# valette/FROG

Hardware: AMD Instinct MI355X
Metric: registration iterations/sec (linear+deformable) (higher is better)
Workload: dtype f32

## Files before the change

### frog_amd/csrc/device/frog_hip.hip

```cpp

#include "ctx.h"
#include <hip/hip_ext.h>
#include "prep.h"
#include "k_links.hip.h"
#include "k_stats.hip.h"
#include "k_grid.hip.h"
#include "k_cull.hip.h"
#include "k_ransac.hip.h"
#include "k_reforder.hip.h"
#include "k_refchain.hip.h"
#include "similarity.h"

#include <atomic>
#include <chrono>
#include <cmath>
#include <cstdlib>
#include <random>
#include <limits>
#include <new>

namespace frog {
thread_local std::string g_last_error;
constexpr int BOUNDS_BLOCKS = 256;
void set_last_error(const std::string &s) { g_last_error = s; }
}

using namespace frog;

#define CTX_GUARD(ctx)                                                   \
    do {                                                                 \
        if (!(ctx)) return fail(FROG_E_INVALID, "null context");         \
        FROG_HIP_CHECK(hipSetDevice((ctx)->device));                      \
    } while (0)

__attribute__((constructor)) static void frog_openmp_defaults()
{
    setenv("KMP_AFFINITY", "disabled", 0);
    setenv("KMP_BLOCKTIME", "0", 0);
}

static inline unsigned div_up(size_t a, size_t b) { return (unsigned)((a + b - 1) / b); }

#include <dlfcn.h>
namespace {
struct Roctx {
    int (*push)(const char *) = nullptr;
    int (*pop)() = nullptr;
    Roctx()
    {
        const char *e = getenv("FROG_ROCTX");
        if (!e || !atoi(e)) return;
        for (const char *name : { "librocprofiler-sdk-roctx.so", "librocprofiler-sdk-roctx.so.1", "libroctx64.so", "libroctx64.so.4" }) {
            if (void *h = dlopen(name, RTLD_NOW | RTLD_GLOBAL)) {
                push = (int (*)(const char *))dlsym(h, "roctxRangePushA");
                pop = (int (*)())dlsym(h, "roctxRangePop");
                if (push && pop) return;
                push = nullptr; pop = nullptr;
            }
        }
    }
};
const Roctx &roctx() { static Roctx r; return r; }
const char *const K_GROUP_NAMES[FROG_K_COUNT_] = { "frog:sweep_linear", "frog:sweep_deformable", "frog:scatter", "frog:lattice_step", "frog:transform_points",
                                                    "frog:update_stats", "frog:combine_energy", "frog:cull_check", "frog:sweep_deformable_build_list",
                                                    "frog:sweep_linear_build_list" };
}

struct Span {
    frog_ctx *c; int slot; hipEvent_t a = nullptr, b = nullptr;
    bool attached;
    bool range = false;
    Span(frog_ctx *ctx, int s, bool attach = false) : c(ctx), slot(s), attached(attach)
    {
        if (roctx().push) { roctx().push(K_GROUP_NAMES[s]); range = true; }
        if (!c->profiling || (c->profiling == 2 && s > FROG_K_SWEEP_DEFORMABLE && s != FROG_K_SWEEP_BUILD && s != FROG_K_SWEEP_LINEAR_BUILD)) return;
        const uint64_t seen = c->span_seen[s]++;
        if (c->profiling == 2 && c->profile_stride > 1 && (s == FROG_K_SWEEP_DEFORMABLE || s == FROG_K_SWEEP_LINEAR) && seen % (uint64_t)c->profile_stride != 0) return;
        if (!c->free_events.empty()) { a = c->free_events.back().first; b = c->free_events.back().second; c->free_events.pop_back(); }
        else if (hipEventCreate(&a) != hipSuccess || hipEventCreate(&b) != hipSuccess) { a = b = nullptr; return; }
        if (!attached) (void)hipEventRecord(a, c->stream);
    }
    ~Span()
    {
        if (a) {
            if (!attached) (void)hipEventRecord(b, c->stream);
            c->spans.push_back({ a, b, slot });
        }
        if (range) roctx().pop();
    }
};

template <class T> static int download_points(frog_ctx *ctx, const T *src, float *dst)
{
    std::vector<T> h(ctx->P);
    FROG_HIP_CHECK(hipMemcpyAsync(h.data(), src, h.size() * sizeof(T), hipMemcpyDeviceToHost, ctx->stream));
    FROG_HIP_CHECK(hipStreamSynchronize(ctx->stream));
    for (size_t p = 0; p < ctx->P; p++) {
        const T &v = h[ctx->h_new_of_old[p]];
        dst[3 * p] = v.x; dst[3 * p + 1] = v.y; dst[3 * p + 2] = v.z;
    }
    return FROG_OK;
}

static unsigned sweep_blocks(const frog_ctx *ctx) { return div_up(ctx->n_tiles, 4) * N_XCD; }

static_assert(THRESHOLD_BAND == 1e-4f, "ctx.h frog_ctx::fast_theta spells the band out");

static uint32_t sweep_lds_images(const frog_ctx *ctx)
{
    if (ctx->rec_format.narrow) return 1u << ctx->rec_format.img_bits;
    uint32_t widest = 0;
    for (uint32_t g = 0; g < ctx->n_groups; g++) widest = std::max(widest, ctx->group_begin[g + 1] - ctx->group_begin[g]);
    return widest <= (uint32_t)EMD_LDS_IMAGES ? widest : 0u;
}

static SweepArgs sweep_args(frog_ctx *ctx, uint32_t sub)
{
    SweepArgs a;
    a.sub = sub;
    a.n_groups = ctx->n_groups;
    for (uint32_t g = 0; g <= ctx->n_groups; g++) a.group_begin[g] = ctx->group_begin[g];
    a.tiles = ctx->tiles.p; a.recs = ctx->rec_format.narrow ? (const void *)ctx->recs32.p : (const void *)ctx->recs.p; a.pos2 = ctx->pos2.p; a.emd = ctx->emd.p; a.emf = ctx->emf.p; a.em = ctx->em.p;
    a.rec2_last = (uint32_t)(ctx->L_recs / 2 - 1);
    a.img_bits = ctx->rec_format.img_bits; a.lds_images = sweep_lds_images(ctx); a.poff = ctx->d_poff.p; a.point_last = (uint32_t)(ctx->P ? ctx->P - 1 : 0);
    a.n_tiles = ctx->n_tiles; a.threshold = ctx->opt.inlier_threshold;
    a.band = ctx->exact_weights ? __builtin_inff() : THRESHOLD_BAND;
    a.tile_partial = ctx->tile_partial.p; a.tile_counts = ctx->tile_counts.p; a.group_sums = ctx->group_sums.p;
    a.own_pt_begin = ctx->own_pt_begin; a.own_points = ctx->own_pt_end - ctx->own_pt_begin;
    a.act_recs = nullptr; a.act_cnt = nullptr; a.cull_state = nullptr;
    a.cut_list = nullptr; a.build_recs = nullptr; a.build_cnt = nullptr;
    a.point_sums = ctx->point_sums.p; a.tile_order = ctx->tile_order.p; a.tiles_bo = ctx->tiles_bo.p;
    return a;
}

static bool cull_active(const frog_ctx *ctx)
{
    return ctx->cull_enabled && ctx->deformable && ctx->opt.inlier_threshold >= 1e-3f && ctx->n_tiles > 0;
}

static bool cull_active_linear(const frog_ctx *ctx)
{
    return ctx->cull_enabled && ctx->cull_linear && !ctx->exact_weights && !ctx->deformable && ctx->n_tiles > 0 && ctx->n_sub == 1;
}

static bool sweep_builds_list(const frog_ctx *ctx) { return ctx->rec_format.narrow != 0; }

static bool sweep_fused_now(const frog_ctx *ctx, bool build)
{
    return ctx->fused_sweep && !build;
}

template <int MODE>
static void launch_sweep(frog_ctx *ctx, uint32_t sub, hipStream_t s, hipEvent_t ea = nullptr, hipEvent_t eb = nullptr,
                         bool use_list = false, bool build_list = false)
{
    uint32_t widest = 0;
    for (uint32_t g = 0; g < ctx->n_groups; g++) widest = std::max(widest, ctx->group_begin[g + 1] - ctx->group_begin[g]);
    if (ctx->n_tiles == 0) return;
    SweepArgs args = sweep_args(ctx, sub);
    if (use_list) {
        args.act_recs = ctx->rec_format.narrow ? (const void *)ctx->act_recs32.p : (const void *)ctx->act_recs.p;
        args.act_cnt = ctx->act_cnt.p;
        args.cull_state = ctx->cull_state.p;
    }
    const dim3 grid(sweep_blocks(ctx)), block(256);
    const size_t lds = (size_t)args.lds_images * (sizeof(EmDerived) + sizeof(uint32_t) + sizeof(float));
    if constexpr (MODE == SWEEP_LINEAR) {
        if (build_list && sweep_builds_list(ctx)) {
            args.act_recs = nullptr; args.act_cnt = nullptr;
            args.cut_list = ctx->cut_list.p; args.build_recs = ctx->act_recs32.p; args.build_cnt = ctx->act_cnt.p;
            hipExtLaunchKernelGGL((sweep_kernel<SWEEP_LINEAR, true, false, true>), grid, block, lds, s, ea, eb, 0, args);
            return;
        }
    }
    if constexpr (MODE == SWEEP_DEFORMABLE) {
        const bool build = build_list && sweep_builds_list(ctx);
        if (build) {
            args.act_recs = nullptr; args.act_cnt = nullptr;
            args.cut_list = ctx->cut_list.p; args.build_recs = ctx->act_recs32.p; args.build_cnt = ctx->act_cnt.p;
        }
        if (sweep_fused_now(ctx, build)) {
            const dim3 fgrid(ctx->n_order_blocks), fblock(512);
            const size_t flds = lds * N_XCD;
            if (ctx->rec_format.narrow) hipExtLaunchKernelGGL((sweep_kernel<SWEEP_DEFORMABLE, true, false, false, true>), fgrid, fblock, flds, s, ea, eb, 0, args);
            else hipExtLaunchKernelGGL((sweep_kernel<SWEEP_DEFORMABLE, true, true, false, true>), fgrid, fblock, flds, s, ea, eb, 0, args);
            return;
        }
        if (build) {
            hipExtLaunchKernelGGL((sweep_kernel<SWEEP_DEFORMABLE, true, false, true>), grid, block, lds, s, ea, eb, 0, args);
            return;
        }
    }
    if (ctx->rec_format.narrow)
        hipExtLaunchKernelGGL((sweep_kernel<MODE, true, false>), grid, block, lds, s, ea, eb, 0, args);
    else if (widest <= (uint32_t)EMD_LDS_IMAGES)
        hipExtLaunchKernelGGL((sweep_kernel<MODE, true, true>), grid, block, lds, s, ea, eb, 0, args);
    else
        hipExtLaunchKernelGGL((sweep_kernel<MODE, false, true>), grid, block, 0, s, ea, eb, 0, args);
}

static int cull_allocate(frog_ctx *ctx);
static int cull_prepare(frog_ctx *ctx);
static int make_geometry(const frog_ctx *ctx, int level, const double mins[3], const double maxs[3], GridGeom &g, frog_grid_info &info);
static int lattice_alloc(frog_ctx *ctx, const GridGeom &g);

__global__ void scratch_warm_kernel(unsigned int *out, int n)
{
    volatile unsigned int a[16];
    for (int k = 0; k < 16; k++) a[k] = (unsigned int)(k * n);
    unsigned int v = 0;
    for (int k = 0; k < 16; k++) v += a[(k + n) & 15];
    if (n < 0) out[0] = v;
}

static uint32_t scatter_max_blocks(uint32_t n_bricks_total, uint32_t n_points, uint32_t chunk)
{
    return std::min(n_bricks_total, n_points) + n_points / chunk;
}

static int queue_setup_kernels(frog_ctx *ctx, hipStream_t s)
{
    const GridGeom &g = ctx->geom;
    const uint32_t nO = ctx->n_owned();
    const uint32_t nPts = ctx->own_pt_end - ctx->own_pt_begin;
    const size_t nb = (size_t)g.n_bricks;
    int rc = FROG_OK;
    {
        ZeroList z{};
        auto add = [&](void *p, size_t bytes) {
            if (!p || !bytes) return;
            z.p[z.n] = (uint32_t *)p; z.bytes[z.n] = bytes;
            z.first_block[z.n + 1] = z.first_block[z.n] + (unsigned)((bytes + ZERO_BLOCK_BYTES - 1) / ZERO_BLOCK_BYTES);
            z.n++;
        };
        add(ctx->gradf.p, ctx->gradf.bytes()); add(ctx->coeff.p, ctx->coeff.bytes()); add(ctx->grad.p, ctx->grad.bytes());
        add(ctx->gridsum.p, ctx->gridsum.bytes()); add(ctx->key_counts.p, ctx->key_counts.bytes());
        add(ctx->len_hist.p, ctx->len_hist.bytes());
        if (g.sparse) {
            add(ctx->lat_mask.p, ctx->lat_mask.bytes()); add(ctx->ucoeff.p, ctx->ucoeff.bytes()); add(ctx->ugrad.p, ctx->ugrad.bytes());
            add(ctx->ugrad_spare.p, ctx->ugrad_spare.bytes());
        }
        if (z.n) {
            zero_buffers_kernel<<<z.first_block[z.n], 256, 0, s>>>(z);
            FROG_HIP_CHECK(hipGetLastError());
        }
    }

    const uint32_t keys_per_brick = (uint32_t)(g.brick * g.brick * g.brick);
    const uint32_t n_keys = (uint32_t)((size_t)nO * nb * keys_per_brick);
    const uint32_t n_bricks_total = nO * (uint32_t)nb;
    frog::DevBuf<uint32_t> &counts = ctx->key_counts, &chunks = ctx->brick_ptr_scratch;
    const GeomDev gd = to_dev(g);
    uint32_t max_img_pts = 0;
    for (uint32_t i = ctx->ib; i < ctx->ie; i++) max_img_pts = std::max(max_img_pts, ctx->poff[i + 1] - ctx->poff[i]);
    const dim3 bgrid(std::max(1u, div_up(max_img_pts, BRICK_BLOCK_POINTS)), nO);
    if (nPts) {
        brick_count_kernel<<<bgrid, 256, 0, s>>>(ctx->pos.p, ctx->d_poff.p, ctx->ib, gd, counts.p);
        FROG_HIP_CHECK(hipGetLastError());
    }
    auto exclusive_scan = [&](const uint32_t *in, uint32_t n, uint32_t *ptr, uint32_t *cursor) -> int {
        const uint32_t n_scan_blocks = div_up(n, SCAN_BLOCK_ITEMS);
        frog::DevBuf<uint32_t> &bsums = ctx->scan_sums;
        scan_block_sums_kernel<<<n_scan_blocks, 1024, 0, s>>>(in, n, bsums.p);
        scan_of_sums_kernel<<<1, 1024, 0, s>>>(bsums.p, n_scan_blocks, bsums.p + n_scan_blocks);
        scan_apply_kernel<<<n_scan_blocks, 1024, 0, s>>>(in, n, bsums.p, bsums.p + n_scan_blocks, ptr, cursor);
        FROG_HIP_CHECK(hipGetLastError());
        return FROG_OK;
    };
    rc = exclusive_scan(counts.p, n_keys, ctx->key_ptr.p, ctx->key_cursor.p);
    if (rc) return rc;
    if (nPts) {
        brick_place_kernel<<<bgrid, 256, 0, s>>>(ctx->pos.p, ctx->d_poff.p, ctx->ib, gd, ctx->key_cursor.p, ctx->perm.p, ctx->perm_key.p);
        FROG_HIP_CHECK(hipGetLastError());
        cell_order_kernel<<<div_up(nPts, 256), 256, 0, s>>>(ctx->key_ptr.p, ctx->perm_key.p, nPts, ctx->perm.p, ctx->perm_tmp.p);
        FROG_HIP_CHECK(hipGetLastError());
        std::swap(ctx->perm.p, ctx->perm_tmp.p);
        std::swap(ctx->perm.cap, ctx->perm_tmp.cap);
        std::swap(ctx->perm.n, ctx->perm_tmp.n);
        gather_positions_kernel<<<div_up(nPts, 256), 256, 0, s>>>(ctx->pos.p, ctx->perm.p, nPts, ctx->pos_b.p);
        FROG_HIP_CHECK(hipGetLastError());
        ctx->pos_b_stale = false;
    }
    const uint32_t max_blocks = scatter_max_blocks(n_bricks_total, nPts, SCATTER_CHUNK);
    brick_chunks_kernel<<<div_up(n_bricks_total, 256), 256, 0, s>>>(ctx->key_ptr.p, n_bricks_total, keys_per_brick, SCATTER_CHUNK, chunks.p);
    FROG_HIP_CHECK(hipGetLastError());
    rc = exclusive_scan(chunks.p, n_bricks_total, ctx->brick_slot_ptr.p, ctx->key_cursor.p );
    if (rc) return rc;
    ScatterBlock *blk_tmp = reinterpret_cast<ScatterBlock *>(ctx->scatter_blocks_tmp.p);
    ScatterBlock *blk = reinterpret_cast<ScatterBlock *>(ctx->scatter_blocks.p);
    uint32_t *len_hist = ctx->len_hist.p, *len_cursor = ctx->len_hist.p + (SCATTER_CHUNK + 1);
    const uint32_t *n_blocks_dev = ctx->brick_slot_ptr.p + n_bricks_total;
    block_fill_kernel<<<div_up(n_bricks_total, 256), 256, 0, s>>>(ctx->key_ptr.p, ctx->brick_slot_ptr.p, n_bricks_total, keys_per_brick,
                                                                 SCATTER_CHUNK, blk_tmp, len_hist);
    static_assert(SCATTER_CHUNK + 1 <= 1024, "block_len_base_kernel: one thread per block length");
    block_len_base_kernel<<<1, (SCATTER_CHUNK + 1 + 63) / 64 * 64, 0, s>>>(len_hist, len_cursor);
    if (max_blocks)
        block_sort_kernel<<<div_up(max_blocks, 256), 256, 0, s>>>(blk_tmp, n_blocks_dev, SCATTER_CHUNK, len_cursor, blk);
    if (g.sparse) {
        if (nPts && max_blocks) lattice_mask_kernel<<<max_blocks, 64, 0, s>>>(ctx->pos_b.p, blk, n_blocks_dev, gd, ctx->lat_mask.p);
        lattice_inactive_kernel<<<div_up((size_t)gd.n_cp, 256), 256, 0, s>>>(ctx->lat_mask.p, nO, gd, ctx->lat_inactive.p);
    }
    FROG_HIP_CHECK(hipGetLastError());
    return FROG_OK;
}

static int join_setup(frog_ctx *ctx)
{
    if (ctx->setup_deferred) {
        ctx->setup_deferred = false;
        FROG_HIP_CHECK(hipStreamWaitEvent(ctx->setup_stream, ctx->setup_fork, 0));
        const int rc = queue_setup_kernels(ctx, ctx->setup_stream);
        if (rc) return rc;
        FROG_HIP_CHECK(hipEventRecord(ctx->setup_join, ctx->setup_stream));
        ctx->setup_pending = true;
    }
    if (!ctx->setup_pending) return FROG_OK;
    FROG_HIP_CHECK(hipStreamWaitEvent(ctx->stream, ctx->setup_join, 0));
    ctx->setup_pending = false;
    return FROG_OK;
}

static int join_setup_positions(frog_ctx *ctx)
{
    const int rc = join_setup(ctx);
    if (rc) return rc;
    const uint32_t nPts = ctx->own_pt_end - ctx->own_pt_begin;
    if (ctx->pos_b_stale && nPts && ctx->pos_b.p && ctx->perm.p) {
        gather_positions_kernel<<<div_up(nPts, 256), 256, 0, ctx->stream>>>(ctx->pos.p, ctx->perm.p, nPts, ctx->pos_b.p);
        FROG_HIP_CHECK(hipGetLastError());
        ctx->pos_b_stale = false;
    }
    return FROG_OK;
}

static int wait_step_scalars(frog_ctx *ctx, double seq)
{
    volatile double *h = ctx->h_energy;
    const auto t0 = std::chrono::steady_clock::now();
    unsigned spins = 0;
    while (h[7] != seq) {
        __builtin_ia32_pause();
        if ((++spins & 0xFFFFu) == 0u && std::chrono::steady_clock::now() - t0 > std::chrono::seconds(20)) {
            FROG_HIP_CHECK(hipStreamSynchronize(ctx->stream));
            if (h[7] != seq) return fail(FROG_E_HIP, "the step's scalars never arrived");
        }
    }
    std::atomic_thread_fence(std::memory_order_acquire);
    return FROG_OK;
}

static int produce_selection(frog_ctx *c)
{
    const int b = (int)(c->sel_produced % (uint64_t)c->sel_ring);
    const uint32_t nO = c->n_owned(), cap = (uint32_t)c->sample_cap;
    if (c->sel_produced >= (uint64_t)c->sel_ring)
        FROG_HIP_CHECK(hipStreamWaitEvent(c->side, c->ord_read[b], 0));
    select_kernel<<<nO, SELECT_THREADS, 0, c->side>>>(c->mt_state.p, c->d_virtual.p, cap, c->sample_ord[b].p, c->sample_count[b].p);
    sample_resolve_kernel<<<dim3(div_up(cap, 256), nO), 256, 0, c->side>>>(
        c->sample_ord[b].p, c->sample_count[b].p, cap, c->d_poff.p, c->ib, c->own_pt_begin,
        c->ref_rowptr.p, c->ref_link.p, c->new_of_old.p, c->sample_ends[b].p);
    FROG_HIP_CHECK(hipGetLastError());
    FROG_HIP_CHECK(hipEventRecord(c->sel_done[b], c->side));
    c->sel_produced++;
    return FROG_OK;
}

static int ref_rows_build(frog_ctx *ctx);
static int ref_alloc(frog_ctx *ctx)
{
    if (ctx->ref_img_link.p) return FROG_OK;
    const uint32_t nO = ctx->n_owned(), nRows = ctx->own_pt_end - ctx->own_pt_begin;
    std::vector<uint64_t> il(nO + 1);
    for (uint32_t i = 0; i <= nO; i++) il[i] = ctx->img_link_begin[ctx->ib + i];
    FROG_HIP_CHECK(ctx->ref_img_link.upload(il, ctx->stream));
    FROG_HIP_CHECK(hipStreamSynchronize(ctx->stream));
    FROG_HIP_CHECK(ctx->ref_own.alloc(std::max<size_t>(1, ctx->L_own)));
    FROG_HIP_CHECK(ctx->ref_link_img.alloc(std::max<size_t>(1, ctx->L_own)));
    FROG_HIP_CHECK(ctx->ref_pt_energy.alloc(2 * (size_t)std::max(1u, nRows)));
    FROG_HIP_CHECK(ctx->ref_row_sums.alloc(std::max(1u, nRows)));
    if (!ctx->ref_stream) {
        FROG_HIP_CHECK(hipStreamCreateWithFlags(&ctx->ref_stream, hipStreamNonBlocking));
        FROG_HIP_CHECK(hipEventCreateWithFlags(&ctx->ref_fork, hipEventDisableTiming));
        FROG_HIP_CHECK(hipEventCreateWithFlags(&ctx->ref_join, hipEventDisableTiming));
    }
    FROG_HIP_CHECK(ctx->ref_w.alloc(std::max<size_t>(1, ctx->L_own)));
    FROG_HIP_CHECK(ctx->ref_d.alloc(std::max<size_t>(1, ctx->L_own)));
    if (nRows)
        ref_link_static_kernel<<<div_up(nRows, 256), 256, 0, ctx->stream>>>(ctx->ref_rowptr.p, ctx->ref_link.p, ctx->new_of_old.p, nRows, ctx->pos.p,
                                                                          ctx->ref_own.p, ctx->ref_link_img.p);
    FROG_HIP_CHECK(hipGetLastError());
    return ctx->ref_literal ? FROG_OK : ref_rows_build(ctx);
}

static int ref_rows_build(frog_ctx *ctx)
{
    if (ctx->rr_valid) return FROG_OK;
    hipStream_t s = ctx->stream;
    const uint32_t nRows = ctx->own_pt_end - ctx->own_pt_begin;
    const uint32_t n_groups = div_up(std::max(1u, nRows), 64u);
    const size_t n_slots = (size_t)n_groups * 64;
    DevBuf<uint32_t> len, len_sorted, iota;
    DevBuf<uint64_t> group_size;
    DevBuf<unsigned char> temp;
    FROG_HIP_CHECK(len.alloc(n_slots)); FROG_HIP_CHECK(len_sorted.alloc(n_slots)); FROG_HIP_CHECK(iota.alloc(n_slots));
    FROG_HIP_CHECK(ctx->rr_slot_row.alloc(n_slots)); FROG_HIP_CHECK(ctx->rr_group_len.alloc(n_groups));
    FROG_HIP_CHECK(group_size.alloc((size_t)n_groups + 1)); FROG_HIP_CHECK(ctx->rr_group_ptr.alloc((size_t)n_groups + 1));
    size_t t1 = 0, t2 = 0;
    FROG_HIP_CHECK(hipcub::DeviceRadixSort::SortPairsDescending(nullptr, t1, len.p, len_sorted.p, iota.p, ctx->rr_slot_row.p, n_slots, 0, 32, s));
    FROG_HIP_CHECK(hipcub::DeviceScan::ExclusiveSum(nullptr, t2, group_size.p, ctx->rr_group_ptr.p, (size_t)n_groups + 1, s));
    FROG_HIP_CHECK(temp.alloc(std::max<size_t>(16, std::max(t1, t2))));
    FROG_HIP_CHECK(hipMemsetAsync(len.p, 0, n_slots * sizeof(uint32_t), s));
    FROG_HIP_CHECK(hipMemsetAsync(iota.p, 0xFF, n_slots * sizeof(uint32_t), s));
    if (nRows) ref_rows_len_kernel<<<div_up(nRows, 256), 256, 0, s>>>(ctx->ref_rowptr.p, nRows, len.p, iota.p);
    size_t tb = temp.n;
    FROG_HIP_CHECK(hipcub::DeviceRadixSort::SortPairsDescending(temp.p, tb, len.p, len_sorted.p, iota.p, ctx->rr_slot_row.p, n_slots, 0, 32, s));
    FROG_HIP_CHECK(hipMemsetAsync(group_size.p, 0, ((size_t)n_groups + 1) * sizeof(uint64_t), s));
    ref_rows_group_kernel<<<div_up(n_groups, 256), 256, 0, s>>>(len_sorted.p, n_groups, ctx->rr_group_len.p, group_size.p);
    tb = temp.n;
    FROG_HIP_CHECK(hipcub::DeviceScan::ExclusiveSum(temp.p, tb, group_size.p, ctx->rr_group_ptr.p, (size_t)n_groups + 1, s));
    uint64_t seats = 0;
    FROG_HIP_CHECK(hipMemcpyAsync(&seats, ctx->rr_group_ptr.p + n_groups, sizeof seats, hipMemcpyDeviceToHost, s));
    FROG_HIP_CHECK(hipStreamSynchronize(s));
    FROG_HIP_CHECK(ctx->rr_ent.alloc(std::max<uint64_t>(1, seats)));
    FROG_HIP_CHECK(ctx->rr_ent_img.alloc(std::max<uint64_t>(1, seats)));
    FROG_HIP_CHECK(hipMemsetAsync(ctx->rr_ent.p, 0xFF, std::max<uint64_t>(1, seats) * sizeof(uint32_t), s));
    FROG_HIP_CHECK(hipMemsetAsync(ctx->rr_ent_img.p, 0, std::max<uint64_t>(1, seats) * sizeof(uint16_t), s));
    ref_rows_fill_kernel<<<n_groups, 64, 0, s>>>(ctx->ref_rowptr.p, ctx->ref_link.p, ctx->pos.p, ctx->rr_slot_row.p, ctx->rr_group_ptr.p,
                                                ctx->rr_ent.p, ctx->rr_ent_img.p);
    FROG_HIP_CHECK(hipGetLastError());
    FROG_HIP_CHECK(hipStreamSynchronize(s));
    ctx->rr_n_groups = n_groups;
    ctx->rr_valid = true;
    return FROG_OK;
}

static int ref_linear_step(frog_ctx *ctx)
{
    { const int rc = ref_alloc(ctx); if (rc) return rc; }
    hipStream_t s = ctx->stream;
    const uint32_t nO = ctx->n_owned(), nRows = ctx->own_pt_end - ctx->own_pt_begin;
    if (ctx->ref_literal) {
        if (nRows)
            ref_link_terms_kernel<<<div_up(nRows, 256), 256, 0, s>>>(ctx->ref_rowptr.p, ctx->ref_link.p, ctx->new_of_old.p, nRows, ctx->pos.p,
                                                                     ctx->pos2.p, ctx->em.p, ctx->ref_own.p, ctx->ref_w.p, ctx->ref_d.p);
        ref_linear_chain_kernel<<<nO, 64, 0, s>>>(ctx->ref_img_link.p, ctx->ref_link.p, ctx->ref_own.p, ctx->ref_w.p, ctx->ref_d.p, ctx->pos2.p,
                                                  ctx->ib, ctx->mat.p, ctx->opt.linear_alpha, ctx->opt.use_scale, ctx->img_energy.p);
    } else if (nO) {
        uint64_t longest = 0;
        for (uint32_t i = ctx->ib; i < ctx->ie; i++) longest = std::max(longest, ctx->img_link_begin[i + 1] - ctx->img_link_begin[i]);
        if (longest)
            ref_link_weights_kernel<<<dim3(div_up(longest, 64 * RW_UNROLL), nO), 64, 0, s>>>(ctx->ref_img_link.p, ctx->ref_link.p, ctx->ref_own.p,
                                                                                            ctx->ref_link_img.p, ctx->pos2.p, ctx->em.p, ctx->emd.p,
                                                                                            ctx->ib, ctx->ref_w.p, ctx->ref_d.p);
        ref_linear_chain2_kernel<<<nO, 64 * (RL_PRODUCERS + 1), 0, s>>>(ctx->ref_img_link.p, ctx->ref_link.p, ctx->ref_own.p, ctx->ref_w.p, ctx->ref_d.p,
                                                                       ctx->pos2.p, ctx->ib, ctx->mat.p, ctx->opt.linear_alpha,
                                                                       ctx->opt.use_scale, ctx->img_energy.p);
    }
    ref_energy_total_kernel<<<1, 1, 0, s>>>(ctx->img_energy.p, nO, ctx->energy.p);
    FROG_HIP_CHECK(hipGetLastError());
    return FROG_OK;
}

static int ref_point_sums(frog_ctx *ctx, bool with_energy)
{
    { const int rc = ref_alloc(ctx); if (rc) return rc; }
    hipStream_t s = ctx->stream;
    const uint32_t nO = ctx->n_owned(), nRows = ctx->own_pt_end - ctx->own_pt_begin;
    if (nRows && ctx->ref_literal) {
        ref_point_sums_kernel<<<div_up(nRows, 256), 256, 0, s>>>(ctx->ref_rowptr.p, ctx->ref_link.p, ctx->new_of_old.p, nRows, ctx->pos.p,
                                                                 ctx->pos2.p, ctx->em.p, ctx->opt.inlier_threshold, ctx->point_sums.p,
                                                                 with_energy ? ctx->ref_pt_energy.p : nullptr);
    } else if (nRows) {
        const int rc = ref_rows_build(ctx);
        if (rc) return rc;
        ref_point_sums_rows_kernel<<<ctx->rr_n_groups, 64, 0, s>>>(ctx->rr_ent.p, ctx->rr_ent_img.p, ctx->rr_group_ptr.p, ctx->rr_group_len.p,
                                                                  ctx->rr_slot_row.p, ctx->new_of_old.p, ctx->pos.p, ctx->pos2.p, ctx->em.p,
                                                                  ctx->emd.p, ctx->opt.inlier_threshold, ctx->point_sums.p, ctx->n_hard ? nullptr : ctx->ref_row_sums.p,
                                                                  with_energy ? ctx->ref_pt_energy.p : nullptr);
    }
    ctx->point_sums_stale = false;
    if (with_energy) {
        hipStream_t se = s;
        if (!ctx->ref_literal && !ctx->n_hard && ctx->ref_stream) {
            FROG_HIP_CHECK(hipEventRecord(ctx->ref_fork, s));
            FROG_HIP_CHECK(hipStreamWaitEvent(ctx->ref_stream, ctx->ref_fork, 0));
            se = ctx->ref_stream;
// ... 2217 lines not shown
```

### frog_amd/csrc/device/k_links.hip.h

```cpp
#pragma once

#include "ctx.h"

#include <type_traits>

namespace frog {

enum { SWEEP_LINEAR = 0, SWEEP_DEFORMABLE = 1, SWEEP_COUNT = 2 };
constexpr int CHUNK_RING = 3, CHUNK_AHEAD = 2;
constexpr int PT_RING = 3, PT_AHEAD = 2;
constexpr int BODY_STEPS = 6;
static_assert(BODY_STEPS == 2 * CHUNK_RING && BODY_STEPS % PT_RING == 0 && PT_AHEAD < PT_RING && CHUNK_AHEAD < CHUNK_RING
              && 2 * CHUNK_AHEAD >= PT_AHEAD + 2, "ring periods must divide the unrolled body; a gather needs its record");
constexpr int EMD_LDS_IMAGES = 256;
constexpr uint32_t CULL_DUP_BIT = 0x80000000u;
constexpr int OWNER_WORDS = TILE_POINTS / 2;
static_assert((OWNER_WORDS & (OWNER_WORDS - 1)) == 0, "the election word of a point is its index masked");
static_assert(EMD_LDS_IMAGES == 1 << 8, "prep.h admits narrow records for img_bits <= 8 only");
constexpr int LINEAR_SUMS = 18;

struct SweepArgs {
    const Tile *tiles;
    const void *recs;
    const uint32_t *poff;
    uint32_t img_bits;
    uint32_t lds_images;
    uint32_t point_last;
    const P3 *pos2;
    const EmDerived *emd;
    const EmFast *emf;
    const float4 *em;
    uint32_t n_tiles;
    uint32_t rec2_last;
    float threshold;
    float band;
    double *tile_partial;
    long long *tile_counts;
    float4 *group_sums;
    float4 *point_sums;
    const uint32_t *tile_order;
    const Tile *tiles_bo;
    uint32_t own_pt_begin, own_points;
    uint32_t sub;
    uint32_t n_groups;
    uint32_t group_begin[MAX_GROUPS + 1];
    const void *act_recs;
    const uint32_t *act_cnt;
    const uint32_t *cull_state;
    const float *cut_list;
    void *build_recs;
    uint32_t *build_cnt;
};


__device__ __forceinline__ float sqrt_rn(float x)
{
    const float s = __builtin_amdgcn_sqrtf(x);
    const float lo = __uint_as_float(__float_as_uint(s) - 1u), hi = __uint_as_float(__float_as_uint(s) + 1u);
    const float e_lo = __builtin_fmaf(-lo, s, x), e_hi = __builtin_fmaf(-hi, s, x);
    float r = (0.0f >= e_lo) ? lo : s;
    r = (0.0f < e_hi) ? hi : r;
    return r;
}

__device__ __forceinline__ float div_fast(float n, float d)
{
    float r = __builtin_amdgcn_rcpf(d);
    r = __builtin_fmaf(__builtin_fmaf(-d, r, 1.0f), r, r);
    return n * r;
}

constexpr float THRESHOLD_BAND = 1e-4f;
__device__ __forceinline__ float chi_pdf_exact(float x)
{
    const float c = 0.797884560802865f;
    const float x2 = x * x;
    return (float)((double)(c * x2) * exp(-0.5 * (double)x2));
}
__device__ __noinline__ float inlier_probability_exact(float d, const float4 em)
{
    const float eps = 1e-10f;
    if (d < 0.1f) return 1.0f;
    const float c1 = em.x + eps, c2 = em.y + eps;
    const float x1 = em.z * chi_pdf_exact(d / c1) / c1;
    const float x2 = (float)((1.0 - (double)em.z) * (double)chi_pdf_exact(d / c2) / (double)c2);
    return x1 / (x1 + x2 + eps);
}

constexpr float INLIER_PROBABILITY_BOUND = 1.52587890625e-05f;
constexpr float D2_FIX = __builtin_bit_cast(float, 0x3c23d70au);
__device__ __forceinline__ float inlier_probability(float d2, const EmDerived e)
{
    const float e1 = __builtin_amdgcn_exp2f(d2 * e.s1), e2 = __builtin_amdgcn_exp2f(d2 * e.s2);
    const float x1 = e.kq1 * (d2 * e1), x2 = e.kq2 * (d2 * e2);
    const float p = div_fast(x1, x1 + x2 + 1e-10f);
    return d2 < D2_FIX ? 1.0f : p;
}

__device__ __forceinline__ float inlier_weight_pair(float d2, const EmFast a, const EmFast b, bool &in_range)
{
    const float e = fmaxf(__builtin_fmaf(a.ds, d2, a.l), __builtin_fmaf(b.ds, d2, b.l));
    in_range = d2 >= b.lo && d2 <= b.hi;
    return __builtin_amdgcn_rcpf(1.0f + __builtin_amdgcn_exp2f(e));
}

__device__ __forceinline__ double wave_sum(double v)
{
    #pragma unroll
    for (int off = 32; off > 0; off >>= 1) v += __shfl_down(v, off, 64);
    return v;
}

__device__ __forceinline__ long long wave_sum_ll(long long v)
{
    #pragma unroll
    for (int off = 32; off > 0; off >>= 1) v += __shfl_down(v, off, 64);
    return v;
}

#ifdef FROG_SWEEP_TRACE
__device__ unsigned long long g_sweep_trace[8 * 8 * 16384];
#define FROG_TR(slot) do { if constexpr (FUSED && !BUILD) { if (lane == 0 && blockIdx.x < 16384) g_sweep_trace[((size_t)blockIdx.x * 8 + wave) * 8 + (slot)] = wall_clock64(); } } while (0)
#else
#define FROG_TR(slot) do { } while (0)
#endif

template <int MODE, bool EMD_LDS, bool WIDE, bool BUILD = false, bool FUSED = false>
__global__ __launch_bounds__(FUSED ? 512 : 256, 1) void sweep_kernel(const SweepArgs a)
{
    static_assert(!(BUILD && FUSED), "the fused sweep does not write the culling list");
    static_assert(!BUILD || (MODE != SWEEP_COUNT && EMD_LDS && !WIDE), "the list is built by the narrow linear / deformable sweeps");
    static_assert(!FUSED || (MODE == SWEEP_DEFORMABLE && EMD_LDS), "the fused form is the deformable sweep's");
    constexpr int WAVES = FUSED ? 8 : 4;
    constexpr int OWN_TILES = FUSED ? 1 : 4;
    __shared__ float4 acc[(MODE == SWEEP_DEFORMABLE) ? WAVES * TILE_POINTS : 1];
    __shared__ unsigned int owner[(MODE == SWEEP_DEFORMABLE) ? WAVES * OWNER_WORDS : 1];
    __shared__ float own_xyz[3 * OWN_TILES * TILE_POINTS];
    extern __shared__ __align__(16) unsigned char sweep_dyn_lds[];
    const int wave = threadIdx.x >> 6;
    const int lane = threadIdx.x & 63;
    unsigned char *tables = sweep_dyn_lds + (FUSED ? (size_t)wave * a.lds_images * (sizeof(EmDerived) + 2 * sizeof(uint32_t)) : (size_t)0);
    EmDerived *emd_s = reinterpret_cast<EmDerived *>(tables);
    EmFast *emf_s = reinterpret_cast<EmFast *>(tables);
    static_assert(sizeof(EmFast) == sizeof(EmDerived), "the two tables share their place");
    constexpr bool W1 = MODE == SWEEP_DEFORMABLE;
    uint32_t *img_base_s = reinterpret_cast<uint32_t *>(tables + (size_t)a.lds_images * sizeof(EmDerived));
    float *cut_s = reinterpret_cast<float *>(img_base_s + a.lds_images);
    __shared__ uint32_t last_step_s[BUILD ? WAVES * TILE_POINTS : 1];

    FROG_TR(0);
    const uint32_t xcd = FUSED ? (uint32_t)wave : blockIdx.x % N_XCD;
    const uint32_t grp = FUSED ? (uint32_t)wave : a.sub * N_XCD + xcd;
    const uint32_t t = FUSED ? a.tile_order[blockIdx.x] : (blockIdx.x / N_XCD) * 4 + wave;
    const bool live = t < a.n_tiles;

    uint32_t pt_begin = 0, pt_count = 0, rec_lo = 0, rec_n = 0, image = 0;
    if (FUSED || live) {
        const Tile &tl = FUSED ? a.tiles_bo[blockIdx.x] : a.tiles[t];
        pt_begin = tl.pt_begin; pt_count = tl.pt_count; image = tl.image;
        rec_lo = tl.rec_begin + tl.group_off[grp];
        rec_n = tl.group_cnt[grp];
    }
    bool listed = false;
    if constexpr (MODE != SWEEP_COUNT) listed = a.act_cnt != nullptr && a.cull_state[0] == 0u;
    bool elect = true;
    if (listed && live) {
        const uint32_t c = a.act_cnt[(size_t)t * a.n_groups + grp];
        rec_n = c & ~CULL_DUP_BIT;
        elect = (c & CULL_DUP_BIT) != 0u;
    }
    elect = __builtin_amdgcn_readfirstlane((uint32_t)elect) != 0u;
    rec_lo = __builtin_amdgcn_readfirstlane(rec_lo);
    rec_n = __builtin_amdgcn_readfirstlane(rec_n);
    pt_begin = __builtin_amdgcn_readfirstlane(pt_begin);
    pt_count = __builtin_amdgcn_readfirstlane(pt_count);
    image = __builtin_amdgcn_readfirstlane(image);
    float4 *my = acc + (MODE == SWEEP_DEFORMABLE ? wave * TILE_POINTS : 0);
    unsigned int *own = owner + (MODE == SWEEP_DEFORMABLE ? wave * OWNER_WORDS : 0);

    if (MODE == SWEEP_DEFORMABLE) {
        for (int k = lane; k < TILE_POINTS; k += 64) {
            my[k] = (a.sub > 0 && (uint32_t)k < pt_count) ? a.group_sums[group_sum_index(xcd, pt_begin - a.own_pt_begin + k, a.own_points)]
                                                          : make_float4(0.f, 0.f, 0.f, 0.f);
            if (k < OWNER_WORDS) own[k] = 0xFFFFFFFFu;
        }
    }
    typedef unsigned long long v2u64 __attribute__((ext_vector_type(2)));
    typedef unsigned int v2u32 __attribute__((ext_vector_type(2)));
    using Rec = std::conditional_t<WIDE, unsigned long long, unsigned int>;
    using Chunk = std::conditional_t<WIDE, v2u64, v2u32>;
    const Chunk *rec2 = reinterpret_cast<const Chunk *>(listed ? a.act_recs : a.recs);
    const uint32_t rec2_lo = rec_lo / 2u + lane;
    auto chunk_at = [&](uint32_t c) { return __builtin_nontemporal_load(rec2 + min(rec2_lo + c * (REC_CHUNK / 2), a.rec2_last)); };
    FROG_TR(1);
    Chunk cq_first[CHUNK_AHEAD];
    #pragma unroll
    for (int k = 0; k < CHUNK_AHEAD; k++) cq_first[k] = chunk_at(k);

    float *px = own_xyz + (FUSED ? 0 : wave * TILE_POINTS);
    constexpr int PLANE = OWN_TILES * TILE_POINTS;
    if constexpr (FUSED) {
        for (uint32_t k = threadIdx.x; k < pt_count; k += 64 * WAVES) {
            const P3 p = a.pos2[pt_begin + k];
            px[k] = p.x; px[k + PLANE] = p.y; px[k + 2 * PLANE] = p.z;
        }
    } else {
        for (uint32_t k = lane; k < pt_count; k += 64) {
            const P3 p = a.pos2[pt_begin + k];
            px[k] = p.x; px[k + PLANE] = p.y; px[k + 2 * PLANE] = p.z;
        }
    }
    const uint32_t g_first = a.group_begin[grp], g_count = a.group_begin[grp + 1] - g_first;
    const uint32_t fill_id = FUSED ? (uint32_t)lane : threadIdx.x, fill_stride = FUSED ? 64u : 256u;
    if (EMD_LDS) {
        if constexpr (W1) {
            const EmFast fO = a.emf[image];
            for (uint32_t k = fill_id; k < g_count; k += fill_stride) {
                EmFast f = a.emf[g_first + k];
                if constexpr (FUSED) { f.lo = fmaxf(f.lo, fO.lo); f.hi = fminf(f.hi, fO.hi); }
                emf_s[k] = f;
            }
        }
        else { for (uint32_t k = fill_id; k < g_count; k += fill_stride) emd_s[k] = a.emd[g_first + k]; }
    }
    if (!WIDE)
        for (uint32_t k = fill_id; k < a.lds_images; k += fill_stride) img_base_s[k] = k < g_count ? a.poff[g_first + k] : 0u;
    uint32_t *last_step = last_step_s + (BUILD ? wave * TILE_POINTS : 0);
    if constexpr (BUILD) {
        for (uint32_t k = fill_id; k < a.lds_images; k += fill_stride) cut_s[k] = k < g_count ? a.cut_list[g_first + k] : 0.f;
        for (int k = lane; k < TILE_POINTS; k += 64) last_step[k] = 0xFFFFFFFFu;
    }
    __syncthreads();
    FROG_TR(2);
    const float cutA = BUILD ? a.cut_list[image] : 0.f;
    uint32_t built = 0;
    bool dup = false;

    const EmDerived eA = a.emd[image];
    const EmFast fA = a.emf[image];

    double s[(MODE == SWEEP_LINEAR) ? LINEAR_SUMS : 2];
    #pragma unroll
    for (int k = 0; k < ((MODE == SWEEP_LINEAR) ? LINEAR_SUMS : 2); k++) s[k] = 0.0;
    long long n_in = 0, n_out = 0;

    const uint32_t img_bits = a.img_bits;
    auto own_of = [&](Rec rq) { return (uint32_t)rq & 0xFFu; };
    auto img_of = [&](Rec rq) {
        if constexpr (WIDE) return ((uint32_t)rq >> 8) - (EMD_LDS ? g_first : 0u);
        else return __builtin_amdgcn_ubfe((uint32_t)rq, 8u, img_bits);
    };
    auto gather = [&](Rec rq) {
        if constexpr (WIDE) return a.pos2[(uint32_t)(rq >> 32)];
        else return a.pos2[min(img_base_s[img_of(rq)] + ((uint32_t)rq >> (8u + img_bits)), a.point_last)];
    };
    Chunk cq[CHUNK_RING];
    P3 pbq[PT_RING];
    #pragma unroll
    for (int k = 0; k < CHUNK_RING; k++) cq[k] = (k < CHUNK_AHEAD) ? cq_first[k < CHUNK_AHEAD ? k : 0] : Chunk{ 0, 0 };
    #pragma unroll
    for (int k = 0; k < PT_RING; k++) pbq[k] = (k < PT_AHEAD) ? gather((k & 1) ? cq[k / 2].y : cq[k / 2].x) : P3{ 0.f, 0.f, 0.f };

    auto step = [&](const Rec rq, const P3 pb, auto elect_c, const bool valid) __attribute__((always_inline)) {
        constexpr bool ELECT = decltype(elect_c)::value;
        const uint32_t ia = own_of(rq);
        const P3 pa = { px[ia], px[ia + PLANE], px[ia + 2 * PLANE] };
        EmDerived eB;
        EmFast fB;
        if constexpr (W1) {
            fB = EMD_LDS ? emf_s[img_of(rq)] : a.emf[img_of(rq)];
            if constexpr (!(EMD_LDS && FUSED)) { fB.lo = fmaxf(fB.lo, fA.lo); fB.hi = fminf(fB.hi, fA.hi); }
        }
        else eB = EMD_LDS ? emd_s[img_of(rq)] : a.emd[img_of(rq)];

        const float dx = pb.x - pa.x, dy = pb.y - pa.y, dz = pb.z - pa.z;
        const float d2 = dx * dx + dy * dy + dz * dz;
        if constexpr (BUILD) {
            const float cut = fminf(cutA, cut_s[img_of(rq)]);
            const bool keep = valid && !(d2 >= cut * cut);
            const unsigned long long m = __ballot(keep);
            if (keep) {
                const uint32_t to = built + (uint32_t)__popcll(m & ((1ull << lane) - 1ull));
                reinterpret_cast<Rec *>(a.build_recs)[(size_t)rec_lo + (to / REC_CHUNK) * REC_CHUNK + (to % 64u) * 2u + (to % REC_CHUNK) / 64u] = rq;
                dup |= atomicExch(&last_step[ia], to >> 6) == (to >> 6);
            }
            built += (uint32_t)__popcll(m);
            if (!valid) return;
        }
        float w;
        if constexpr (W1) {
            bool in_range;
            w = inlier_weight_pair(d2, fA, fB, in_range);
            asm volatile("" : "+v"(w));
            if (!in_range && !(w < a.threshold - a.band)) {
                const uint32_t imgB = img_of(rq) + (WIDE && !EMD_LDS ? 0u : g_first);
                w = fminf(inlier_probability(d2, eA), inlier_probability(d2, a.emd[imgB]));
            }
        } else w = fminf(inlier_probability(d2, eA), inlier_probability(d2, eB));
        if constexpr (MODE != SWEEP_LINEAR) {
            if (fabsf(w - a.threshold) < a.band) {
                const uint32_t imgB = img_of(rq) + (WIDE && !EMD_LDS ? 0u : g_first);
                const float d = sqrt_rn(d2);
                w = fminf(inlier_probability_exact(d, a.em[image]), inlier_probability_exact(d, a.em[imgB]));
            }
        } else if (a.band > 1.0f) {
            const uint32_t imgB = img_of(rq) + (WIDE && !EMD_LDS ? 0u : g_first);
            const float d = sqrt_rn(d2);
            w = fminf(inlier_probability_exact(d, a.em[image]), inlier_probability_exact(d, a.em[imgB]));
        }

        if constexpr (MODE == SWEEP_LINEAR) {
            const float d = sqrt_rn(d2);
            s[16] += (double)(w * w * d * d);
            s[17] += (double)(w * w);
            s[0] += (double)(w * dx); s[1] += (double)(w * dy); s[2] += (double)(w * dz);
            s[3] += (double)(w * pa.x); s[4] += (double)(w * pa.y); s[5] += (double)(w * pa.z);
            s[6] += (double)(w * pb.x); s[7] += (double)(w * pb.y); s[8] += (double)(w * pb.z);
            s[9] += (double)(w * pa.x * pa.x); s[10] += (double)(w * pa.y * pa.y); s[11] += (double)(w * pa.z * pa.z);
            s[12] += (double)(w * pb.x * pb.x); s[13] += (double)(w * pb.y * pb.y); s[14] += (double)(w * pb.z * pb.z);
            s[15] += (double)w;
        } else if constexpr (MODE == SWEEP_DEFORMABLE) {
            const bool inlier = w >= a.threshold;
            const float w2 = w * w;
            s[1] += (double)(inlier ? w2 : 0.0f);
            s[0] += (double)(inlier ? w2 * d2 : 0.0f);
            if constexpr (!ELECT) {
                if (inlier) {
                    float4 t = my[ia];
                    t.x += w2 * dx; t.y += w2 * dy; t.z += w2 * dz; t.w += w2;
                    my[ia] = t;
                }
                __builtin_amdgcn_fence(__ATOMIC_RELEASE, "wavefront");
                __builtin_amdgcn_wave_barrier();
                return;
            }
            bool pending = inlier;
            const uint32_t io = ia & (OWNER_WORDS - 1);
            while (__ballot(pending)) {
                if (pending) atomicMin(&own[io], (unsigned int)lane);
                __builtin_amdgcn_fence(__ATOMIC_RELEASE, "wavefront");
                __builtin_amdgcn_wave_barrier();
                if (pending && __hip_atomic_load(&own[io], __ATOMIC_RELAXED, __HIP_MEMORY_SCOPE_WAVEFRONT) == (unsigned int)lane) {
                    float4 t = my[ia];
                    t.x += w2 * dx; t.y += w2 * dy; t.z += w2 * dz; t.w += w2;
                    my[ia] = t;
                    own[io] = 0xFFFFFFFFu;
                    pending = false;
                }
                __builtin_amdgcn_fence(__ATOMIC_RELEASE, "wavefront");
                __builtin_amdgcn_wave_barrier();
            }
        } else {
            if (w < a.threshold) n_out++; else n_in++;
        }
    };

    const uint32_t n_steps = (rec_n + 63) / 64;
    auto walk = [&](auto elect_c) __attribute__((always_inline)) {
        for (uint32_t base = 0; base < n_steps; base += BODY_STEPS) {
            #pragma unroll
            for (int j = 0; j < BODY_STEPS; j++) {
                const uint32_t r = lane + 64 * (base + j);
                if (j % 2 == 0) cq[(j / 2 + CHUNK_AHEAD) % CHUNK_RING] = chunk_at(base / 2 + j / 2 + CHUNK_AHEAD);
                {
                    const Chunk ahead = cq[((j + PT_AHEAD) / 2) % CHUNK_RING];
                    pbq[(j + PT_AHEAD) % PT_RING] = gather(((j + PT_AHEAD) & 1) ? ahead.y : ahead.x);
                }
                if (BUILD || r < rec_n) step((j & 1) ? cq[j / 2].y : cq[j / 2].x, pbq[j % PT_RING], elect_c, r < rec_n);
#ifdef FROG_SWEEP_TRACE
                if (base == 0 && j == 0) FROG_TR(3);
#endif
            }
        }
    };
    if (MODE != SWEEP_DEFORMABLE || elect) walk(std::true_type{});
    else walk(std::false_type{});
    FROG_TR(4);

    if constexpr (BUILD) {
        const uint32_t cap = (rec_n + REC_CHUNK - 1) / REC_CHUNK * REC_CHUNK;
        const uint32_t reach = (((built + 63u) / 64u + BODY_STEPS - 1u) / BODY_STEPS * BODY_STEPS + PT_AHEAD) * 64u;
        for (uint32_t k = built + lane; k < min(cap, reach); k += 64)
            reinterpret_cast<Rec *>(a.build_recs)[(size_t)rec_lo + (k / REC_CHUNK) * REC_CHUNK + (k % 64u) * 2u + (k % REC_CHUNK) / 64u] = (Rec)0;
    }
    if constexpr (MODE == SWEEP_LINEAR) {
        #pragma unroll
        for (int k = 0; k < LINEAR_SUMS; k++) {
            double v = wave_sum(s[k]);
            if (lane == 0 && live) a.tile_partial[((size_t)t * a.n_groups + grp) * LINEAR_SUMS + k] = v;
        }
        if constexpr (BUILD) {
            if (lane == 0 && live) a.build_cnt[(size_t)t * a.n_groups + grp] = built | CULL_DUP_BIT;
        }
    } else if constexpr (MODE == SWEEP_DEFORMABLE) {
        double v0 = wave_sum(s[0]), v1 = wave_sum(s[1]);
        if (lane == 0 && live) {
            a.tile_partial[((size_t)t * a.n_groups + grp) * 2] = v0;
            a.tile_partial[((size_t)t * a.n_groups + grp) * 2 + 1] = v1;
        }
        if constexpr (BUILD) {
            const bool any_dup = __ballot(dup) != 0ull;
            if (lane == 0 && live) a.build_cnt[(size_t)t * a.n_groups + grp] = built | (any_dup ? CULL_DUP_BIT : 0u);
        }
        __syncthreads();
        FROG_TR(5);
        typedef float v4f __attribute__((ext_vector_type(4)));
        if constexpr (FUSED) {
            for (uint32_t k = threadIdx.x; k < pt_count; k += 64 * WAVES) {
                float4 v = acc[k];
                #pragma unroll
                for (int g = 1; g < N_XCD; g++) {
                    const float4 u = acc[g * TILE_POINTS + k];
                    v.x += u.x; v.y += u.y; v.z += u.z; v.w += u.w;
                }
                a.point_sums[pt_begin + k] = v;
            }
#ifdef FROG_SWEEP_TRACE
            if constexpr (!BUILD) { if (lane == 0 && blockIdx.x < 16384) { g_sweep_trace[((size_t)blockIdx.x * 8 + wave) * 8 + 6] = wall_clock64(); g_sweep_trace[((size_t)blockIdx.x * 8 + wave) * 8 + 7] = rec_n; } }
#endif
        } else {
            for (uint32_t k = lane; k < pt_count; k += 64) {
                const float4 v = my[k];
                float4 *dst = a.group_sums + group_sum_index(xcd, pt_begin - a.own_pt_begin + k, a.own_points);
                __builtin_nontemporal_store((v4f){ v.x, v.y, v.z, v.w }, reinterpret_cast<v4f *>(dst));
            }
        }
    } else {
        long long v0 = wave_sum_ll(n_in), v1 = wave_sum_ll(n_out);
        if (lane == 0 && live) {
            a.tile_counts[((size_t)t * a.n_groups + grp) * 2] = v0;
            a.tile_counts[((size_t)t * a.n_groups + grp) * 2 + 1] = v1;
        }
    }
}

__global__ __launch_bounds__(256) void combine_groups_kernel(const float4 *group_sums, uint32_t own_points,
                                                             uint32_t own_pt_begin, float4 *point_sums)
{
    const uint32_t i = blockIdx.x * blockDim.x + threadIdx.x;
    if (i >= own_points) return;
    float4 s = group_sums[group_sum_index(0, i, own_points)];
    #pragma unroll
    for (int g = 1; g < N_XCD; g++) {
        const float4 v = group_sums[group_sum_index(g, i, own_points)];
        s.x += v.x; s.y += v.y; s.z += v.z; s.w += v.w;
    }
    point_sums[own_pt_begin + i] = s;
}

__global__ void hard_links_kernel(const P3 *pos2, float4 *point_sums, const uint32_t *point, const uint32_t *ptr,
                                  const uint32_t *partner, uint32_t n_hard, float w2, double *partial)
{
    const uint32_t t = blockIdx.x * blockDim.x + threadIdx.x;
    if (t >= n_hard) return;
    const uint32_t a = point[t];
    const P3 pA = pos2[a];
    float4 s = point_sums[a];
    double sd = 0, sw = 0;
    for (uint32_t l = ptr[t]; l < ptr[t + 1]; l++) {
        const P3 pB = pos2[partner[l]];
        const float dx = pB.x - pA.x, dy = pB.y - pA.y, dz = pB.z - pA.z;
        const float d2 = dx * dx + dy * dy + dz * dz;
        sd += (double)(w2 * d2);
        sw += (double)w2;
        s.x += w2 * dx; s.y += w2 * dy; s.z += w2 * dz; s.w += w2;
    }
    point_sums[a] = s;
    if (partial) { partial[2 * t] = sd; partial[2 * t + 1] = sw; }
}

__global__ void hard_energy_kernel(const double *partial, uint32_t n_hard, double *energy)
{
    if (blockIdx.x || threadIdx.x) return;
    double a = 0, b = 0;
    for (uint32_t t = 0; t < n_hard; t++) { a += partial[2 * t]; b += partial[2 * t + 1]; }
    energy[0] += a; energy[1] += b;
}

constexpr int ENERGY_BLOCKS = 64;

__global__ __launch_bounds__(256) void energy_reduce_kernel(const double *partial, uint32_t n, int stride, int off,
                                                            double *block_sums , unsigned int *ticket,
                                                            double *energy, const uint32_t *list_invalid = nullptr,
                                                            unsigned int *stray = nullptr)
{
    __shared__ double sh[2][256];
    __shared__ bool last;
    const uint32_t per = (n + gridDim.x - 1) / gridDim.x;
    const uint32_t b = min(n, blockIdx.x * per), e = min(n, b + per);
    double a0 = 0, a1 = 0;
    for (uint32_t t = b + threadIdx.x; t < e; t += 256) {
        a0 += partial[(size_t)t * stride + off];
        a1 += partial[(size_t)t * stride + off + 1];
    }
    sh[0][threadIdx.x] = a0; sh[1][threadIdx.x] = a1;
    __syncthreads();
    for (int h = 128; h > 0; h >>= 1) {
        if ((int)threadIdx.x < h) { sh[0][threadIdx.x] += sh[0][threadIdx.x + h]; sh[1][threadIdx.x] += sh[1][threadIdx.x + h]; }
        __syncthreads();
    }
    if (threadIdx.x == 0) {
        __hip_atomic_store(&block_sums[2 * blockIdx.x], sh[0][0], __ATOMIC_RELAXED, __HIP_MEMORY_SCOPE_AGENT);
        __hip_atomic_store(&block_sums[2 * blockIdx.x + 1], sh[1][0], __ATOMIC_RELAXED, __HIP_MEMORY_SCOPE_AGENT);
        __threadfence();
        last = atomicAdd(ticket, 1u) == gridDim.x - 1;
    }
    __syncthreads();
    if (!last) return;
    __threadfence();
    if (threadIdx.x < 2 * gridDim.x && threadIdx.x < 256)
        sh[0][threadIdx.x] = __hip_atomic_load(&block_sums[threadIdx.x], __ATOMIC_RELAXED, __HIP_MEMORY_SCOPE_AGENT);
    __syncthreads();
    if (threadIdx.x == 0) {
        double s0 = 0, s1 = 0;
        for (unsigned int k = 0; k < gridDim.x; k++) { s0 += sh[0][2 * k]; s1 += sh[0][2 * k + 1]; }
        energy[0] = s0; energy[1] = s1; energy[2] = 0.0;
        energy[3] = list_invalid ? (double)list_invalid[0] : 0.0;
        if (stray) stray[0] = stray[1] = 0u;
        *ticket = 0u;
    }
}

__global__ __launch_bounds__(256) void linear_update_kernel(const double *partial, const uint32_t *img_tile_ptr,
                                                            uint32_t n_groups, uint32_t image_begin, double *mat,
                                                            float linear_alpha, int use_scale,
                                                            double *img_energy = nullptr, unsigned int *ticket = nullptr,
                                                            double *energy = nullptr, const uint32_t *list_invalid = nullptr)
{
    __shared__ double part[8][32];
    __shared__ double sums[LINEAR_SUMS];
    __shared__ bool last_s;
    const uint32_t image = image_begin + blockIdx.x;
    const uint32_t t0 = img_tile_ptr[image] * n_groups, t1 = img_tile_ptr[image + 1] * n_groups;
    const int comp = threadIdx.x & 31, slice = threadIdx.x >> 5;
    if (comp < LINEAR_SUMS) {
        double v = 0;
        for (uint32_t t = t0 + slice; t < t1; t += 64) {
            double w[8];
            #pragma unroll
            for (int u = 0; u < 8; u++) w[u] = (t + 8u * u < t1) ? partial[(size_t)(t + 8u * u) * LINEAR_SUMS + comp] : 0.0;
            #pragma unroll
            for (int u = 0; u < 8; u++) v += w[u];
        }
        part[slice][comp] = v;
    }
    __syncthreads();
    if (threadIdx.x < LINEAR_SUMS) {
        double v = 0;
        for (int sl = 0; sl < 8; sl++) v += part[sl][threadIdx.x];
        sums[threadIdx.x] = v;
    }
    __syncthreads();
    if (threadIdx.x < 3) {
        const int k = threadIdx.x;
        double *M = mat + (size_t)image * 16;
        const double sDisp = sums[k], sPosA = sums[3 + k], sPosB = sums[6 + k];
        const double sPosA2 = sums[9 + k], sPosB2 = sums[12 + k], sWeight = sums[15];
        const float scale = (float)M[5 * k];
        float newScale = 1.0f;
        if (use_scale)
            newScale = (float)pow((sWeight * sPosB2 - sPosB * sPosB) / (sWeight * sPosA2 - sPosA * sPosA),
                                  0.5 * (double)linear_alpha);
        if (!isnan(newScale)) {
            M[5 * k] = (double)(scale * newScale);
            const float translation = (float)M[4 * k + 3];
            if (!isnan(translation))
                M[4 * k + 3] = (double)translation + (double)linear_alpha * sDisp / sWeight
                             + sPosA * (double)(1 - newScale) / sWeight;
        }
    }
    if (!img_energy) return;
    if (threadIdx.x == 0) {
        __hip_atomic_store(&img_energy[2 * blockIdx.x], sums[16], __ATOMIC_RELAXED, __HIP_MEMORY_SCOPE_AGENT);
        __hip_atomic_store(&img_energy[2 * blockIdx.x + 1], sums[17], __ATOMIC_RELAXED, __HIP_MEMORY_SCOPE_AGENT);
        __threadfence();
        last_s = atomicAdd(ticket, 1u) == gridDim.x - 1;
    }
    __syncthreads();
    if (!last_s) return;
    __threadfence();
    __shared__ double pairs_s[2][256];
    double s0 = 0, s1 = 0;
    for (uint32_t base = 0; base < gridDim.x; base += 256) {
        const uint32_t i = base + threadIdx.x;
        if (i < gridDim.x) {
            pairs_s[0][threadIdx.x] = __hip_atomic_load(&img_energy[2 * i], __ATOMIC_RELAXED, __HIP_MEMORY_SCOPE_AGENT);
            pairs_s[1][threadIdx.x] = __hip_atomic_load(&img_energy[2 * i + 1], __ATOMIC_RELAXED, __HIP_MEMORY_SCOPE_AGENT);
        }
        __syncthreads();
        if (threadIdx.x == 0)
            for (uint32_t k = 0; k < min(256u, gridDim.x - base); k++) { s0 += pairs_s[0][k]; s1 += pairs_s[1][k]; }
        __syncthreads();
    }
    if (threadIdx.x == 0) {
        energy[0] = s0; energy[1] = s1; energy[2] = 0.0;
        energy[3] = list_invalid ? (double)list_invalid[0] : 0.0;
        *ticket = 0u;
    }
}

__global__ void count_reduce_kernel(const long long *tile_counts, const uint32_t *img_tile_ptr, uint32_t n_groups,
                                    uint32_t image_begin, uint32_t n_owned, long long *out )
{
    uint32_t i = blockIdx.x * blockDim.x + threadIdx.x;
    if (i >= n_owned) return;
    const uint32_t image = image_begin + i;
    long long a = 0, b = 0;
    for (uint32_t t = img_tile_ptr[image] * n_groups; t < img_tile_ptr[image + 1] * n_groups; t++) { a += tile_counts[(size_t)t * 2]; b += tile_counts[(size_t)t * 2 + 1]; }
    out[(size_t)i * 2] = a; out[(size_t)i * 2 + 1] = b;
}

}
```

Baseline: 2416.

## Shrink fused sweep LDS and let the last-arriving wave reduce the point sums

The fused deformable sweep now sizes its per-wave dynamic LDS tables exactly, dropping the unused cut slot and the image-base slot for wide records and padding to 16 bytes. Pairs of waves share one owner-election array, using workgroup-scope atomics and a wave-tagged id, which halves that array. The block-wide barrier before the cross-wave reduction is replaced by an arrival counter, so only the last wave to finish sums the eight accumulators while the others exit early. The aim is lower LDS per block for more resident blocks and less idle waiting at the barrier, at the cost of more contention on the shared owner words and a reduction done by a single wave. A FROG_TIMING-gated occupancy printout is also added.

```diff
diff --git a/frog_amd/csrc/device/frog_hip.hip b/frog_amd/csrc/device/frog_hip.hip
--- a/frog_amd/csrc/device/frog_hip.hip
+++ b/frog_amd/csrc/device/frog_hip.hip
@@ -181,7 +181,19 @@
         }
         if (sweep_fused_now(ctx, build)) {
             const dim3 fgrid(ctx->n_order_blocks), fblock(512);
-            const size_t flds = lds * N_XCD;
+            const size_t flds = (size_t)fused_table_bytes(args.lds_images, !ctx->rec_format.narrow) * N_XCD;
+            const void *fn = ctx->rec_format.narrow ? (const void *)sweep_kernel<SWEEP_DEFORMABLE, true, false, false, true>
+                                                    : (const void *)sweep_kernel<SWEEP_DEFORMABLE, true, true, false, true>;
+            static const bool say = getenv("FROG_TIMING") != nullptr;
+            static bool said = false;
+            if (say && !said) {
+                said = true;
+                hipFuncAttributes fa{};
+                int resident = 0;
+                if (hipFuncGetAttributes(&fa, fn) == hipSuccess && hipOccupancyMaxActiveBlocksPerMultiprocessor(&resident, fn, 512, flds) == hipSuccess)
+                    std::printf("[timing] fused sweep: LDS per block %zu B (%zu static + %zu tables), %d registers, %d resident blocks per CU\n",
+                                fa.sharedSizeBytes + flds, fa.sharedSizeBytes, flds, fa.numRegs, resident);
+            }
             if (ctx->rec_format.narrow) hipExtLaunchKernelGGL((sweep_kernel<SWEEP_DEFORMABLE, true, false, false, true>), fgrid, fblock, flds, s, ea, eb, 0, args);
             else hipExtLaunchKernelGGL((sweep_kernel<SWEEP_DEFORMABLE, true, true, false, true>), fgrid, fblock, flds, s, ea, eb, 0, args);
             return;
diff --git a/frog_amd/csrc/device/k_links.hip.h b/frog_amd/csrc/device/k_links.hip.h
--- a/frog_amd/csrc/device/k_links.hip.h
+++ b/frog_amd/csrc/device/k_links.hip.h
@@ -17,6 +17,10 @@
 constexpr int OWNER_WORDS = TILE_POINTS / 2;
 static_assert((OWNER_WORDS & (OWNER_WORDS - 1)) == 0, "the election word of a point is its index masked");
 static_assert(EMD_LDS_IMAGES == 1 << 8, "prep.h admits narrow records for img_bits <= 8 only");
+__host__ __device__ inline uint32_t fused_table_bytes(uint32_t lds_images, bool wide)
+{
+    return (lds_images * (uint32_t)(sizeof(EmFast) + (wide ? 0 : sizeof(uint32_t))) + 15u) & ~15u;
+}
 constexpr int LINEAR_SUMS = 18;
 
 struct SweepArgs {
@@ -134,12 +138,14 @@
     constexpr int WAVES = FUSED ? 8 : 4;
     constexpr int OWN_TILES = FUSED ? 1 : 4;
     __shared__ float4 acc[(MODE == SWEEP_DEFORMABLE) ? WAVES * TILE_POINTS : 1];
-    __shared__ unsigned int owner[(MODE == SWEEP_DEFORMABLE) ? WAVES * OWNER_WORDS : 1];
+    constexpr int OWNER_SETS = FUSED ? WAVES / 2 : WAVES;
+    __shared__ unsigned int owner[(MODE == SWEEP_DEFORMABLE) ? OWNER_SETS * OWNER_WORDS : 1];
+    __shared__ unsigned int arrived_s;
     __shared__ float own_xyz[3 * OWN_TILES * TILE_POINTS];
     extern __shared__ __align__(16) unsigned char sweep_dyn_lds[];
     const int wave = threadIdx.x >> 6;
     const int lane = threadIdx.x & 63;
-    unsigned char *tables = sweep_dyn_lds + (FUSED ? (size_t)wave * a.lds_images * (sizeof(EmDerived) + 2 * sizeof(uint32_t)) : (size_t)0);
+    unsigned char *tables = sweep_dyn_lds + (FUSED ? (size_t)wave * fused_table_bytes(a.lds_images, WIDE) : (size_t)0);
     EmDerived *emd_s = reinterpret_cast<EmDerived *>(tables);
     EmFast *emf_s = reinterpret_cast<EmFast *>(tables);
     static_assert(sizeof(EmFast) == sizeof(EmDerived), "the two tables share their place");
@@ -176,7 +182,8 @@
     pt_count = __builtin_amdgcn_readfirstlane(pt_count);
     image = __builtin_amdgcn_readfirstlane(image);
     float4 *my = acc + (MODE == SWEEP_DEFORMABLE ? wave * TILE_POINTS : 0);
-    unsigned int *own = owner + (MODE == SWEEP_DEFORMABLE ? wave * OWNER_WORDS : 0);
+    unsigned int *own = owner + (MODE == SWEEP_DEFORMABLE ? (FUSED ? wave / 2 : wave) * OWNER_WORDS : 0);
+    const unsigned int bid = FUSED ? (unsigned int)lane | ((unsigned int)wave & 1u) << 6 : (unsigned int)lane;
 
     if (MODE == SWEEP_DEFORMABLE) {
         for (int k = lane; k < TILE_POINTS; k += 64) {
@@ -230,6 +237,7 @@
         for (uint32_t k = fill_id; k < a.lds_images; k += fill_stride) cut_s[k] = k < g_count ? a.cut_list[g_first + k] : 0.f;
         for (int k = lane; k < TILE_POINTS; k += 64) last_step[k] = 0xFFFFFFFFu;
     }
+    if constexpr (FUSED) { if (threadIdx.x == 0) arrived_s = 0u; }
     __syncthreads();
     FROG_TR(2);
     const float cutA = BUILD ? a.cut_list[image] : 0.f;
@@ -337,14 +345,20 @@
             bool pending = inlier;
             const uint32_t io = ia & (OWNER_WORDS - 1);
             while (__ballot(pending)) {
-                if (pending) atomicMin(&own[io], (unsigned int)lane);
+                if (pending) atomicMin(&own[io], bid);
                 __builtin_amdgcn_fence(__ATOMIC_RELEASE, "wavefront");
                 __builtin_amdgcn_wave_barrier();
-                if (pending && __hip_atomic_load(&own[io], __ATOMIC_RELAXED, __HIP_MEMORY_SCOPE_WAVEFRONT) == (unsigned int)lane) {
+                unsigned int holder = 0xFFFFFFFFu;
+                if (pending) {
+                    if constexpr (FUSED) holder = __hip_atomic_load(&own[io], __ATOMIC_RELAXED, __HIP_MEMORY_SCOPE_WORKGROUP);
+                    else holder = __hip_atomic_load(&own[io], __ATOMIC_RELAXED, __HIP_MEMORY_SCOPE_WAVEFRONT);
+                }
+                if (pending && holder == bid) {
                     float4 t = my[ia];
                     t.x += w2 * dx; t.y += w2 * dy; t.z += w2 * dz; t.w += w2;
                     my[ia] = t;
-                    own[io] = 0xFFFFFFFFu;
+                    if constexpr (FUSED) __hip_atomic_store(&own[io], 0xFFFFFFFFu, __ATOMIC_RELAXED, __HIP_MEMORY_SCOPE_WORKGROUP);
+                    else own[io] = 0xFFFFFFFFu;
                     pending = false;
                 }
                 __builtin_amdgcn_fence(__ATOMIC_RELEASE, "wavefront");
@@ -402,11 +416,19 @@
             const bool any_dup = __ballot(dup) != 0ull;
             if (lane == 0 && live) a.build_cnt[(size_t)t * a.n_groups + grp] = built | (any_dup ? CULL_DUP_BIT : 0u);
         }
-        __syncthreads();
         FROG_TR(5);
         typedef float v4f __attribute__((ext_vector_type(4)));
         if constexpr (FUSED) {
-            for (uint32_t k = threadIdx.x; k < pt_count; k += 64 * WAVES) {
+#ifdef FROG_SWEEP_TRACE
+            if constexpr (!BUILD) { if (lane == 0 && blockIdx.x < 16384) { g_sweep_trace[((size_t)blockIdx.x * 8 + wave) * 8 + 6] = 0ull; g_sweep_trace[((size_t)blockIdx.x * 8 + wave) * 8 + 7] = rec_n; } }
+#endif
+            __builtin_amdgcn_fence(__ATOMIC_RELEASE, "workgroup");
+            unsigned int before = 0u;
+            if (lane == 0) before = __hip_atomic_fetch_add(&arrived_s, 1u, __ATOMIC_RELAXED, __HIP_MEMORY_SCOPE_WORKGROUP);
+            before = __builtin_amdgcn_readfirstlane(before);
+            if (before != (unsigned int)(WAVES - 1)) return;
+            __builtin_amdgcn_fence(__ATOMIC_ACQUIRE, "workgroup");
+            for (uint32_t k = lane; k < pt_count; k += 64) {
                 float4 v = acc[k];
                 #pragma unroll
                 for (int g = 1; g < N_XCD; g++) {
@@ -416,7 +438,7 @@
                 a.point_sums[pt_begin + k] = v;
             }
 #ifdef FROG_SWEEP_TRACE
-            if constexpr (!BUILD) { if (lane == 0 && blockIdx.x < 16384) { g_sweep_trace[((size_t)blockIdx.x * 8 + wave) * 8 + 6] = wall_clock64(); g_sweep_trace[((size_t)blockIdx.x * 8 + wave) * 8 + 7] = rec_n; } }
+            if constexpr (!BUILD) { if (lane == 0 && blockIdx.x < 16384) g_sweep_trace[((size_t)blockIdx.x * 8 + wave) * 8 + 6] = wall_clock64(); }
 #endif
         } else {
             for (uint32_t k = lane; k < pt_count; k += 64) {
```

New measurement: 2311. -4.4%, worse.
